# eragonruan/text-detection-ctpn

Hardware: NVIDIA H100
Metric: images/sec @600x900 (higher is better)
Workload: dtype fp32-faithful: fp16 operands + e4m3 cross terms (1 fp16 + 1 e4m3 wgmma per 16 MACs: 2 bf16-rate units per MAC), fp32 accumulate; matmuls around the BiLSTM on bf16x2

## Files before the change

text-detection-ctpn_b200/csrc/conv1_tc.cu:

```cuda
#include <mutex>

#include "common.cuh"
#include "tc_ptx.cuh"

namespace ctpn {

#ifdef CTPN_DEBUG
#define C1_DBG(p, bit) (((p).debug & (bit)) != 0)
#else
#define C1_DBG(p, bit) false
#endif


constexpr int kC1tThreads = 512;
constexpr int kC1tTileBytes = 128 * 128;
constexpr int kC1tPatch = 3 * 18 * 40;

struct Conv1TcParams {
  const void *src;
  const float *lut, *w, *bias;
  __nv_bfloat16 *out;
  int B, H, W, src_is_f32;
  int tiles_x, tiles_y, total_tiles;
  int debug;
  long long plane_stride;
  float out_s, out_t, out_rs;
  const int *sizes;
};

__device__ __forceinline__ void c1_extent(const Conv1TcParams &p, int b, int &eh, int &ew) {
  eh = p.H; ew = p.W;
  if (p.sizes) {
    eh = min(eh, __ldg(p.sizes + 2 * b));
    ew = min(ew, __ldg(p.sizes + 2 * b + 1));
  }
}

template <int P, int OUTQ>
__global__ void __launch_bounds__(kC1tThreads, 1)
conv1_tc_kernel(const Conv1TcParams p) {
  using namespace ptx;
  extern __shared__ uint8_t smem_raw[];
  const uint32_t raw = smem_u32(smem_raw);
  constexpr int kSPG = P <= 2 ? 2 : 1;
  constexpr int kStages = 2 * kSPG;
  const uint32_t a0 = (raw + 1023u) & ~1023u;
  const uint32_t b0 = a0 + (uint32_t)kStages * P * kC1tTileBytes;
  uint8_t *base = smem_raw + (a0 - raw);
  uint8_t *bsm = base + kStages * P * kC1tTileBytes;
  float *patch = reinterpret_cast<float *>(bsm + P * 64 * 128);
  float *lut_s = patch + 4 * kC1tPatch;
  float *epi = lut_s + 768;
  uint64_t *bars = reinterpret_cast<uint64_t *>(epi + 2 * 128 * 32);
  const uint32_t fullA = smem_u32(bars), emptyA = fullA + 32;

  const int warp = __shfl_sync(0xffffffffu, (int)(threadIdx.x >> 5), 0), lane = threadIdx.x & 31;
  if (threadIdx.x == 0) {
    for (int i = 0; i < 4; ++i) {
      mbar_init(fullA + 8 * i, 128);
      mbar_init(emptyA + 8 * i, 2);
    }
    fence_mbar_init();
  }
  if (!p.src_is_f32)
    for (int i = threadIdx.x; i < 768; i += kC1tThreads) lut_s[i] = p.lut[i];
  for (int i = threadIdx.x; i < 64 * 4; i += kC1tThreads) {
    const int co = i >> 2, chunk = i & 3;
    uint32_t pk[3][4];
#pragma unroll
    for (int j = 0; j < 4; ++j) {
      float v[2];
#pragma unroll
      for (int e = 0; e < 2; ++e) {
        const int k = chunk * 8 + j * 2 + e;
        v[e] = k < 27 ? p.w[k * 64 + co] : (k == 27 ? p.bias[co] : 0.f);
      }
      uint32_t t[P];
      split_planes2<P>(v[0], v[1], t);
#pragma unroll
      for (int pl = 0; pl < P; ++pl) pk[pl][j] = t[pl];
    }
#pragma unroll
    for (int pl = 0; pl < P; ++pl)
      *reinterpret_cast<uint4 *>(bsm + pl * 64 * 128 + co * 128 + ((chunk ^ (co & 7)) << 4)) = make_uint4(pk[pl][0], pk[pl][1], pk[pl][2], pk[pl][3]);
  }
  fence_proxy_async();
  __syncthreads();
  const int tiles_per_img = p.tiles_x * p.tiles_y;

  if (warp < 8) {
    const int grp = warp >> 2;
    const int m = (warp & 3) * 32 + lane, th = m >> 3, tw = m & 7;
    const unsigned tpi = (unsigned)tiles_per_img, tx = (unsigned)p.tiles_x;
    uint32_t raw[2][3];
    unsigned valid = 0;
    auto fetch = [&](int tile) {
      valid = 0;
      if (tile >= p.total_tiles) return;
      const unsigned b = (unsigned)tile / tpi, r = (unsigned)tile % tpi;
      const int y0 = (int)(r / tx) * 16, x0 = (int)(r % tx) * 8;
      int eh, ew;
      c1_extent(p, (int)b, eh, ew);
#pragma unroll
      for (int u = 0; u < 2; ++u) {
        const int i = m + u * 128;
        const int xx = i % 10, yy = i / 10;
        const int gx = x0 + xx - 1, gy = y0 + yy - 1;
        if (i < 180 && gx >= 0 && gx < ew && gy >= 0 && gy < eh && !C1_DBG(p, 1)) {
          const size_t off = (((size_t)b * p.H + gy) * p.W + gx) * 3;
          if (p.src_is_f32) {
            const float *q = reinterpret_cast<const float *>(p.src) + off;
            raw[u][0] = __float_as_uint(q[0]); raw[u][1] = __float_as_uint(q[1]); raw[u][2] = __float_as_uint(q[2]);
          } else {
            const uint8_t *q = reinterpret_cast<const uint8_t *>(p.src) + off;
            raw[u][0] = q[0]; raw[u][1] = q[1]; raw[u][2] = q[2];
          }
          valid |= 1u << u;
        }
      }
    };
    fetch(blockIdx.x + grp * gridDim.x);
    int n = 0;
    for (int tile = blockIdx.x + grp * gridDim.x; tile < p.total_tiles; tile += 2 * gridDim.x, ++n) {
      const int s = grp * kSPG + n % kSPG;
      const uint32_t ph = (uint32_t)(n / kSPG) & 1u;
      float *pt = patch + (grp * 2 + (n & 1)) * kC1tPatch;
#pragma unroll
      for (int u = 0; u < 2; ++u) {
        const int i = m + u * 128;
        if (i < 180) {
          const int xx = i % 10, yy = i / 10;
          float v0 = 0.f, v1 = 0.f, v2 = 0.f;
          if ((valid >> u) & 1u) {
            if (p.src_is_f32) {
              v0 = __uint_as_float(raw[u][0]); v1 = __uint_as_float(raw[u][1]); v2 = __uint_as_float(raw[u][2]);
            } else {
              v0 = lut_s[raw[u][0] * 3 + 0]; v1 = lut_s[raw[u][1] * 3 + 1]; v2 = lut_s[raw[u][2] * 3 + 2];
            }
          }
          pt[(0 * 18 + yy) * 40 + xx] = v0;
          pt[(1 * 18 + yy) * 40 + xx] = v1;
          pt[(2 * 18 + yy) * 40 + xx] = v2;
        }
      }
      fetch(tile + 2 * gridDim.x);
      mbar_wait(emptyA + 8 * s, ph ^ 1u);
      if (grp == 0) asm volatile("bar.sync 1, 128;" ::: "memory");
      else asm volatile("bar.sync 2, 128;" ::: "memory");
      uint8_t *arow = base + s * P * kC1tTileBytes + m * 128;
#pragma unroll
      for (int chunk = 0; chunk < (C1_DBG(p, 2) ? 0 : 4); ++chunk) {
        uint32_t pk[3][4];
#pragma unroll
        for (int j = 0; j < 4; ++j) {
          float v[2];
#pragma unroll
          for (int e = 0; e < 2; ++e) {
            const int k = chunk * 8 + j * 2 + e;
            v[e] = k < 27 ? pt[((k % 3) * 18 + th + k / 9) * 40 + tw + (k / 3) % 3] : (k == 27 ? 1.f : 0.f);
          }
          uint32_t t[P];
          split_planes2<P>(v[0], v[1], t);
#pragma unroll
          for (int pl = 0; pl < P; ++pl) pk[pl][j] = t[pl];
        }
#pragma unroll
        for (int pl = 0; pl < P; ++pl)
          *reinterpret_cast<uint4 *>(arow + pl * kC1tTileBytes + ((chunk ^ (m & 7)) << 4)) = make_uint4(pk[pl][0], pk[pl][1], pk[pl][2], pk[pl][3]);
      }
      fence_proxy_async();
      mbar_arrive(fullA + 8 * s);
    }
  } else {
    const int wg = (warp >> 2) - 2;
    const int cw = warp - 8, chunk = cw >> 2, quarter = cw & 3;
    const int m = quarter * 32 + lane, th = m >> 3, tw = m & 7;
    const int frow = wg * 64 + (warp & 3) * 16 + (lane >> 2);
    constexpr uint32_t kHi = gmma_desc_hi(1024);
    const uint32_t b_lo = gmma_desc_lo(b0);
    float accm[32], accc[32];
    uint4 *stage_w = reinterpret_cast<uint4 *>(epi + chunk * 4096 + quarter * 1024);
    int n = 0;
    for (int tile = blockIdx.x; tile < p.total_tiles; tile += gridDim.x, ++n) {
      const int s = (n & 1) * kSPG + (n >> 1) % kSPG;
      const uint32_t ph = (uint32_t)((n >> 1) / kSPG) & 1u;
      const unsigned b = (unsigned)tile / (unsigned)tiles_per_img, r = (unsigned)tile % (unsigned)tiles_per_img;
      const int y = (int)(r / (unsigned)p.tiles_x) * 16 + th, x = (int)(r % (unsigned)p.tiles_x) * 8 + tw;
      const bool ok = y < p.H && x < p.W;
      int eh, ew;
      c1_extent(p, (int)b, eh, ew);
      const bool live = y < eh && x < ew;
      const long long pix = ((long long)b * p.H + y) * p.W + x;
      const unsigned okmask = __ballot_sync(0xffffffffu, ok);
      long long spix[4];
#pragma unroll
      for (int it = 0; it < 4; ++it) {
        const long long hi = __shfl_sync(0xffffffffu, (int)(pix >> 32), it * 8 + (lane >> 2));
        const unsigned lo = __shfl_sync(0xffffffffu, (unsigned)(pix & 0xffffffffll), it * 8 + (lane >> 2));
        spix[it] = (hi << 32) | lo;
      }
      mbar_wait(fullA + 8 * s, ph);
      const uint32_t a_lo = gmma_desc_lo(a0 + s * P * kC1tTileBytes + wg * 64 * 128);
      wgmma_fence();
#pragma unroll
      for (int i = 0; i < P; ++i)
#pragma unroll
        for (int j = 0; j < P - i; ++j)
#pragma unroll
          for (int k = 0; k < 2; ++k) {
            const uint64_t da = ((uint64_t)kHi << 32) | (a_lo + i * (kC1tTileBytes >> 4) + 2u * k);
            const uint64_t db = ((uint64_t)kHi << 32) | (b_lo + j * ((64 * 128) >> 4) + 2u * k);
            if (i + j == 0) wgmma_bf16(accm, da, db, (uint32_t)k);
            else wgmma_bf16(accc, da, db, (k == 0 && i == 0 && j == 1) ? 0u : 1u);
          }
      wgmma_commit();
      wgmma_wait<0>();
      wgmma_fence_regs(accm);
      if (P > 1) wgmma_fence_regs(accc);
      if ((threadIdx.x & 127) == 0) mbar_arrive(emptyA + 8 * s);
      if (P > 1) {
#pragma unroll
        for (int i = 0; i < 32; ++i) accm[i] = accm[i] + accc[i];
      }
      named_sync(3, 256);
#pragma unroll
      for (int j = 0; j < 8; ++j) {
        const int q = 2 * (j & 3) + ((lane & 3) >> 1);
#pragma unroll
        for (int h = 0; h < 2; ++h) {
          const int row = frow + 8 * h;
          *reinterpret_cast<float2 *>(epi + (j >> 2) * 4096 + row * 32 + ((q ^ (row & 7)) << 2) + 2 * (lane & 1)) =
              make_float2(accm[4 * j + 2 * h], accm[4 * j + 2 * h + 1]);
        }
      }
      named_sync(3, 256);
      if (!C1_DBG(p, 8)) {
        float v[32];
#pragma unroll
        for (int q = 0; q < 8; ++q) {
          const float4 t = *reinterpret_cast<const float4 *>(epi + chunk * 4096 + m * 32 + ((q ^ (m & 7)) << 2));
          v[4 * q + 0] = t.x; v[4 * q + 1] = t.y; v[4 * q + 2] = t.z; v[4 * q + 3] = t.w;
        }
        if (!live) {
#pragma unroll
          for (int i = 0; i < 32; ++i) v[i] = 0.f;
        }
        if (OUTQ) {
          uint32_t wh[16], wq[16];
#pragma unroll
          for (int i = 0; i < 8; ++i) {
            const float v0 = fmaxf(v[4 * i], 0.f), v1 = fmaxf(v[4 * i + 1], 0.f), v2 = fmaxf(v[4 * i + 2], 0.f), v3 = fmaxf(v[4 * i + 3], 0.f);
            f16f8_quad(v0, v1, v2, v3, p.out_s, p.out_t, p.out_rs, wh[2 * i], wh[2 * i + 1], wq[i], wq[8 + i]);
          }
#pragma unroll
          for (int pl = 0; pl < 2; ++pl) {
            __syncwarp();
#pragma unroll
            for (int q = 0; q < 4; ++q) {
              const uint4 val = pl == 0 ? make_uint4(wh[4 * q], wh[4 * q + 1], wh[4 * q + 2], wh[4 * q + 3])
                                        : make_uint4(wq[4 * q], wq[4 * q + 1], wq[4 * q + 2], wq[4 * q + 3]);
              stage_w[lane * 4 + (q ^ ((lane >> 1) & 3))] = val;
            }
            __syncwarp();
            uint8_t *obase = reinterpret_cast<uint8_t *>(p.out) + (long long)pl * p.plane_stride * 2;
            const int j = lane & 3;
            const int off = pl == 0 ? chunk * 64 + j * 16 : chunk * 32 + (j >> 1) * 64 + (j & 1) * 16;
#pragma unroll
            for (int it = 0; it < 4; ++it) {
              const int pp = it * 8 + (lane >> 2);
              const uint4 val = stage_w[pp * 4 + (j ^ ((pp >> 1) & 3))];
              if (((okmask >> pp) & 1u) && !C1_DBG(p, 4)) *reinterpret_cast<uint4 *>(obase + spix[it] * 128 + off) = val;
            }
          }
        } else {
        uint32_t w[P][16];
#pragma unroll
        for (int i = 0; i < 16; ++i) {
          uint32_t t[P];
          split_planes2<P>(fmaxf(v[2 * i], 0.f), fmaxf(v[2 * i + 1], 0.f), t);
#pragma unroll
          for (int pl = 0; pl < P; ++pl) w[pl][i] = t[pl];
        }
#pragma unroll
        for (int pl = 0; pl < P; ++pl) {
          __syncwarp();
#pragma unroll
          for (int q = 0; q < 4; ++q) stage_w[lane * 4 + (q ^ ((lane >> 1) & 3))] = make_uint4(w[pl][4 * q], w[pl][4 * q + 1], w[pl][4 * q + 2], w[pl][4 * q + 3]);
          __syncwarp();
          __nv_bfloat16 *obase = p.out + (long long)pl * p.plane_stride + chunk * 32 + (lane & 3) * 8;
#pragma unroll
          for (int it = 0; it < 4; ++it) {
            const int pp = it * 8 + (lane >> 2);
            const uint4 val = stage_w[pp * 4 + ((lane & 3) ^ ((pp >> 1) & 3))];
            if (((okmask >> pp) & 1u) && !C1_DBG(p, 4)) *reinterpret_cast<uint4 *>(obase + spix[it] * 64) = val;
          }
        }
        }
      }
    }
  }
}

template <int P, int OUTQ = 0>
static int launch_conv1_tc(Conv1TcParams &p, cudaStream_t st) {
  const size_t smem = 1024 + (size_t)(P <= 2 ? 4 : 2) * P * kC1tTileBytes + (size_t)P * 64 * 128 +
                      (4 * kC1tPatch + 768 + 2 * 128 * 32) * sizeof(float) + 64;
  constexpr int kMaxDevices = 64;
  static std::mutex mu;
  static int sm_count[kMaxDevices];
  int dev = 0;
  CTPN_CUDA(cudaGetDevice(&dev));
  CTPN_REQUIRE(dev >= 0 && dev < kMaxDevices, "ctpn_conv1_1_tc: device index %d not supported", dev);
  int sms;
  {
    std::lock_guard<std::mutex> lock(mu);
    if (sm_count[dev] == 0) {
      CTPN_CUDA(cudaFuncSetAttribute(conv1_tc_kernel<P, OUTQ>, cudaFuncAttributeMaxDynamicSharedMemorySize, (int)smem));
      CTPN_CUDA(cudaDeviceGetAttribute(&sm_count[dev], cudaDevAttrMultiProcessorCount, dev));
    }
    sms = sm_count[dev];
  }
  const int grid = p.total_tiles < sms ? p.total_tiles : sms;
  ProfScope prof("conv1_1", 2.0 * p.B * p.H * p.W * 27.0 * 64.0, st);
  conv1_tc_kernel<P, OUTQ><<<grid, kC1tThreads, smem, st>>>(p);
  CTPN_LAUNCH_CHECK();
  return CTPN_OK;
}

}

int ctpn::conv1_1_tc_ragged(const void *src, int src_is_f32, const float *lut, const float *w_hwio, const float *bias,
                            void *out_planes, int B, int H, int W, int planes, bool outq, float out_s, float out_t,
                            const int *sizes, void *stream) {
  CTPN_REQUIRE(src && w_hwio && bias && out_planes, "ctpn_conv1_1_tc: null pointer");
  CTPN_REQUIRE(src_is_f32 || lut, "ctpn_conv1_1_tc: uint8 input needs the mean-subtraction LUT");
  CTPN_REQUIRE(B > 0 && H > 0 && W > 0, "ctpn_conv1_1_tc: bad shape");
  CTPN_REQUIRE(planes >= 1 && planes <= 3, "ctpn_conv1_1_tc: planes must be 1..3");
  Conv1TcParams p;
  p.src = src; p.lut = lut; p.w = w_hwio; p.bias = bias; p.out = (__nv_bfloat16 *)out_planes;
  p.B = B; p.H = H; p.W = W; p.src_is_f32 = src_is_f32;
  p.tiles_x = ceil_div(W, 8); p.tiles_y = ceil_div(H, 16);
  const long long total = (long long)B * p.tiles_x * p.tiles_y;
  CTPN_REQUIRE(total < (1ll << 31), "ctpn_conv1_1_tc: too many tiles");
  p.total_tiles = (int)total;
  p.plane_stride = (long long)B * H * W * 64;
  p.out_s = p.out_t = p.out_rs = 1.f;
  p.sizes = sizes;
  if (outq) {
    CTPN_REQUIRE(out_s > 0.f && out_t > 0.f, "ctpn_conv1_1_tc_f16f8: scales must be positive");
    p.out_s = out_s; p.out_t = out_t; p.out_rs = kResidualGain * out_t / out_s;
  }
#ifdef CTPN_DEBUG
  static const int dbg = [] { const char *e = getenv("CTPN_C1_DEBUG"); return e ? atoi(e) : 0; }();
  p.debug = dbg;
#else
  p.debug = 0;
#endif
  cudaStream_t st = (cudaStream_t)stream;
  if (outq) return launch_conv1_tc<2, 1>(p, st);
  if (planes == 1) return launch_conv1_tc<1>(p, st);
  if (planes == 2) return launch_conv1_tc<2>(p, st);
  return launch_conv1_tc<3>(p, st);
}

using namespace ctpn;

extern "C" int ctpn_conv1_1_tc(const void *src, int src_is_f32, const float *lut, const float *w_hwio, const float *bias,
                               void *out_planes, int B, int H, int W, int planes, void *stream) {
  return conv1_1_tc_ragged(src, src_is_f32, lut, w_hwio, bias, out_planes, B, H, W, planes, false, 1.f, 1.f, nullptr, stream);
}

extern "C" int ctpn_conv1_1_tc_f16f8(const void *src, int src_is_f32, const float *lut, const float *w_hwio, const float *bias,
                                     void *out_planes, int B, int H, int W, float out_s, float out_t, void *stream) {
  return conv1_1_tc_ragged(src, src_is_f32, lut, w_hwio, bias, out_planes, B, H, W, 2, true, out_s, out_t, nullptr, stream);
}
```

text-detection-ctpn_b200/csrc/conv_tc.cu:

```cuda
#include <cuda.h>

#include <algorithm>
#include <mutex>
#include <unordered_map>

#include "common.cuh"
#include "tc_ptx.cuh"
#include "tma_host.cuh"

namespace ctpn {

#ifdef CTPN_DEBUG
#define CTPN_DBG(p, bit) (((p).debug & (bit)) != 0)
#else
#define CTPN_DBG(p, bit) false
#endif

struct ConvTcParams {
  int B, H, W, Cin, Cout, taps, planes, flags;
  int tiles_x, tiles_y, tiles_n, total_tiles;
  int m_tiles, total_units;
  int TH, TW, tw_log2;
  int PW;
  int patch_bytes;
// ... 443 lines not shown
#pragma unroll
        for (int i = 0; i < R; ++i)
          accm[i] = F8 ? __fmaf_rn(accc[i], p.inv_cross, accm[i] * p.inv_main) : PR ? __fadd_rn(accs[i], accc[i]) : accm[i] + accc[i];
      }

      if (CTPN_DBG(p, 16)) continue;
      if (EW) {
        const float *bt = p.bias + (u % p.tiles_n) * BN + 2 * (lane & 3);
#pragma unroll
        for (int i8 = 0; i8 < BN / 8; ++i8) {
          const float2 bq = __ldg(reinterpret_cast<const float2 *>(bt + 8 * i8));
#pragma unroll
          for (int h = 0; h < 2; ++h) {
            accm[4 * i8 + 2 * h] += bq.x;
            accm[4 * i8 + 2 * h + 1] += bq.y;
          }
        }
        if (p.flags & CTPN_F_RELU) {
#pragma unroll
          for (int i = 0; i < R; ++i) accm[i] = fmaxf(accm[i], 0.f);
        }
#pragma unroll
        for (int c2 = 0; c2 < BN / 64; ++c2) {
          mbar_wait(epiE, eph ^ 1u);
          stage_half(c2);
          mbar_arrive(epiF);
          eph ^= 1u;
        }
      } else {
        const int cw = warp - 4, eset = cw >> 2, quarter = cw & 3;
        const int m = quarter * 32 + lane;
        int mt, nt;
        unit_tile(u, mt, nt);
        EpiPixel e;
        epi_pixel(p, mt, m, lane, e);
        uint4 *stage_w = reinterpret_cast<uint4 *>(epi + eset * 4096 + quarter * 1024);
#pragma unroll
        for (int c2 = 0; c2 < BN / 64; ++c2) {
          named_sync(1, 256);
          stage_half(c2);
          named_sync(1, 256);
          float v[32];
#pragma unroll
          for (int q = 0; q < 8; ++q) {
            const float4 t = *reinterpret_cast<const float4 *>(epi + eset * 4096 + m * 32 + ((q ^ (m & 7)) << 2));
            v[4 * q + 0] = t.x; v[4 * q + 1] = t.y; v[4 * q + 2] = t.z; v[4 * q + 3] = t.w;
          }
          epi_chunk<P, F8>(p, e, v, nt * BN + (2 * c2 + eset) * 32, stage_w, false, true, lane);
        }
      }
    }
  }
  __syncthreads();
  if (MC) cluster_sync_all();
}


constexpr int kMaxDevices = 64;
static std::mutex g_mu;
static int g_sms[kMaxDevices];

struct Tuning { int debug = 0, bn = 0, stages_a = 0, stages_b = 0, mcast = 1, promote = 1; };
static const Tuning &tuning() {
  static const Tuning t = [] {
    Tuning v;
#ifdef CTPN_DEBUG
    auto env_int = [](const char *name, int dflt) { const char *e = getenv(name); return e ? atoi(e) : dflt; };
    v.debug = env_int("CTPN_TC_DEBUG", 0);
    v.bn = env_int("CTPN_TC_BN", 0);
    v.stages_a = env_int("CTPN_TC_STAGES_A", 0);
    v.stages_b = env_int("CTPN_TC_STAGES_B", 0);
    v.mcast = env_int("CTPN_TC_MCAST", 1);
    v.promote = std::max(1, env_int("CTPN_TC_PROMOTE", 1));
#endif
    return v;
  }();
  return t;
}

struct TmapKey {
  const void *ptr;
  unsigned long long d0, d1, d2, d3;
  unsigned b0, b1, b2, b3;
  int dev;
  bool operator==(const TmapKey &o) const {
    return ptr == o.ptr && d0 == o.d0 && d1 == o.d1 && d2 == o.d2 && d3 == o.d3 && b0 == o.b0 && b1 == o.b1 && b2 == o.b2 &&
           b3 == o.b3 && dev == o.dev;
  }
};
struct TmapKeyHash {
  size_t operator()(const TmapKey &k) const {
    size_t h = std::hash<const void *>()(k.ptr);
    for (unsigned long long v : {k.d0, k.d1, k.d2, k.d3, (unsigned long long)k.b0, (unsigned long long)k.b1,
                                 (unsigned long long)k.b2, (unsigned long long)k.b3, (unsigned long long)k.dev})
      h = h * 1000003u ^ std::hash<unsigned long long>()(v);
    return h;
  }
};
static std::unordered_map<TmapKey, CUtensorMap, TmapKeyHash> g_tmaps;

static int cached_tmap(int dev, CUtensorMap *out, const void *ptr, int rank, const cuuint64_t *dims, const cuuint64_t *strides,
                       const cuuint32_t *box) {
  TmapKey k{ptr, dims[0], dims[1], rank > 2 ? dims[2] : 0, rank > 3 ? dims[3] : 0, box[0], box[1], rank > 2 ? box[2] : 0,
            rank > 3 ? box[3] : 0, dev};
  std::lock_guard<std::mutex> lock(g_mu);
  auto it = g_tmaps.find(k);
  if (it != g_tmaps.end()) { *out = it->second; return CTPN_OK; }
  EncodeTiledFn enc = nullptr;
  int rc = tma_get_encode(&enc);
  if (rc) return rc;
  if ((rc = tma_encode_bf16(enc, out, const_cast<void *>(ptr), rank, dims, strides, box))) return rc;
  if (g_tmaps.size() >= 1024) g_tmaps.clear();
  g_tmaps.emplace(k, *out);
  return CTPN_OK;
}

template <int BN, int P, int TAPS, int MC, int F8 = 0, int PR = 0>
static int launch_bn(int dev, const CUtensorMap &ta, const CUtensorMap &tb, ConvTcParams &p, cudaStream_t st) {
  const size_t a_stage = (size_t)p.planes * p.patch_bytes, b_stage = (size_t)p.planes * BN * 128;
  const size_t epi_bytes = kEpiBytes + (kEpiWarpgroup<BN, PR> ? kXposeBytes : 0);
  const size_t budget = 227 * 1024 - 1024 - kCtrlBytes - epi_bytes;
  int sa = (2 * a_stage + 2 * b_stage <= budget) ? 2 : 1;
  if (p.taps == 1) sa = (int)std::min<size_t>(4, std::max<size_t>(1, (budget / 2) / a_stage));
  CTPN_REQUIRE(sa * a_stage + 2 * b_stage <= budget, "conv_tc: pipeline stages (%zu + 2 x %zu B) do not fit in shared memory", a_stage, b_stage);
  int sb = (int)((budget - sa * a_stage) / b_stage);
  if (sb > kMaxStages) sb = kMaxStages;
  if (tuning().stages_a > 0) sa = std::max(1, std::min(sa, tuning().stages_a));
  if (tuning().stages_b > 0) sb = std::max(2, std::min(sb, tuning().stages_b));
  p.stages_a = sa;
  p.stages_b = sb;
  const size_t smem = 1024 + sa * a_stage + sb * b_stage + epi_bytes + kCtrlBytes;
  CTPN_REQUIRE(smem <= 227 * 1024, "conv_tc: %zu bytes of shared memory", smem);
  auto kernel = conv_tc_kernel<BN, P, TAPS, MC, F8, PR>;
  static bool attr_set[kMaxDevices];
  static int max_clusters[kMaxDevices];
  cudaLaunchConfig_t cfg = {};
  cudaLaunchAttribute attr;
  attr.id = cudaLaunchAttributeClusterDimension;
  attr.val.clusterDim.x = 2; attr.val.clusterDim.y = 1; attr.val.clusterDim.z = 1;
  cfg.blockDim = dim3(kTcThreads<BN, PR>);
  cfg.dynamicSmemBytes = smem;
  cfg.stream = st;
  cfg.attrs = &attr;
  cfg.numAttrs = MC ? 1 : 0;
  {
    std::lock_guard<std::mutex> lock(g_mu);
    if (!attr_set[dev]) {
      CTPN_CUDA(cudaFuncSetAttribute(kernel, cudaFuncAttributeMaxDynamicSharedMemorySize, 227 * 1024));
      if (MC) {
        cfg.gridDim = dim3(2 * (g_sms[dev] / 2));
        int n = 0;
        CTPN_CUDA(cudaOccupancyMaxActiveClusters(&n, kernel, &cfg));
        CTPN_REQUIRE(n > 0, "conv_tc: no 2-CTA cluster of this kernel fits on the device");
        max_clusters[dev] = n;
      }
      attr_set[dev] = true;
    }
  }
  char label[128];
  if (prof_enabled()) snprintf(label, sizeof(label), "conv_tc t%d %dx%dx%d c%d-%d %s%d bn%d%s%s", p.taps, p.B, p.H, p.W, p.Cin, p.Cout, F8 ? "f16f8 p" : "p", p.planes, BN, MC ? " mc" : "", PR ? " promote" : "");
  ProfScope prof(label, p.work, st);
  if (MC) cfg.gridDim = dim3(2 * std::min(max_clusters[dev], p.total_units));
  else cfg.gridDim = dim3(std::min(p.total_units, g_sms[dev]));
  CTPN_CUDA(cudaLaunchKernelEx(&cfg, kernel, ta, tb, p));
  CTPN_LAUNCH_CHECK();
  return CTPN_OK;
}

int conv_tc_run(const void *in_planes, const void *w_planes, const float *bias, void *out, int B, int H, int W, int cin,
                int cout, int taps, int planes, int flags, const QuantScales *q, const int *ext, int ext_shift, void *stream) {
  const bool f8 = q != nullptr, promote = (flags & CTPN_F_PROMOTE) != 0;
  CTPN_REQUIRE(f8 || !(flags & CTPN_F_OUT_BF16X2), "ctpn_conv3x3: CTPN_F_OUT_BF16X2 is a flag of ctpn_conv3x3_f16f8");
  CTPN_REQUIRE(!(promote && f8), "ctpn_conv3x3_f16f8: CTPN_F_PROMOTE is a flag of ctpn_conv3x3 with planes = 3");
  CTPN_REQUIRE(!promote || planes == 3, "ctpn_conv3x3: CTPN_F_PROMOTE needs planes = 3 (got %d)", planes);
  CTPN_REQUIRE(in_planes && w_planes && bias && out, "ctpn_conv3x3: null pointer");
  CTPN_REQUIRE(taps == 9 || taps == 1, "ctpn_conv3x3: taps must be 9 or 1 (got %d)", taps);
  CTPN_REQUIRE(planes >= 1 && planes <= 3, "ctpn_conv3x3: planes must be 1..3 (got %d)", planes);
  CTPN_REQUIRE(cin % 64 == 0 && cin >= 64, "ctpn_conv3x3: Cin must be a multiple of 64 (got %d)", cin);
  CTPN_REQUIRE(cout % 64 == 0 && cout >= 64, "ctpn_conv3x3: Cout must be a multiple of 64 (got %d)", cout);
  CTPN_REQUIRE(B > 0 && H > 0 && W > 0, "ctpn_conv3x3: bad shape");
  const bool pool = flags & CTPN_F_POOL;
  CTPN_REQUIRE(!pool || (taps == 9 && H >= 2 && W >= 2), "ctpn_conv3x3: pooling needs taps=9 and H,W >= 2");
  const bool stack_in = flags & CTPN_F_STACK_IN, stack_out = flags & CTPN_F_STACK_OUT;
  CTPN_REQUIRE(!stack_in || (taps == 9 && !pool), "ctpn_conv3x3: CTPN_F_STACK_IN needs taps=9 and no pooling");
  CTPN_REQUIRE(!stack_out || !(flags & CTPN_F_OUT_F32), "ctpn_conv3x3: stacked output is a plane format");
  const int img_B = B, img_H = H;
  if (stack_in) {
    CTPN_REQUIRE((long long)B * (H + 1) < (1ll << 30), "ctpn_conv3x3: stack too tall");
    H = B * (H + 1);
    B = 1;
  }
  int dev = 0, rc;
  CTPN_CUDA(cudaGetDevice(&dev));
  CTPN_REQUIRE(dev >= 0 && dev < kMaxDevices, "ctpn_conv3x3: device index %d not supported", dev);
// ... 130 lines not shown
```

text-detection-ctpn_b200/csrc/tc_ptx.cuh:

```cuda
#pragma once
#include <cuda.h>
#include <stdint.h>

namespace ctpn {
namespace ptx {

__device__ __forceinline__ uint32_t smem_u32(const void *p) {
  return static_cast<uint32_t>(__cvta_generic_to_shared(p));
}

__device__ __forceinline__ bool elect_one() {
  uint32_t pred = 0;
  asm volatile(
      "{\n\t.reg .pred p;\n\t"
      "elect.sync _|p, 0xffffffff;\n\t"
      "selp.u32 %0, 1, 0, p;\n\t}"
      : "=r"(pred));
  return pred != 0;
}

__device__ __forceinline__ void mbar_init(uint32_t bar, uint32_t count) {
  asm volatile("mbarrier.init.shared::cta.b64 [%0], %1;" ::"r"(bar), "r"(count) : "memory");
}
__device__ __forceinline__ void fence_mbar_init() {
  asm volatile("fence.mbarrier_init.release.cluster;" ::: "memory");
}
__device__ __forceinline__ void fence_proxy_async() {
  asm volatile("fence.proxy.async.shared::cta;" ::: "memory");
}
__device__ __forceinline__ void mbar_arrive_expect_tx(uint32_t bar, uint32_t bytes) {
  asm volatile("mbarrier.arrive.expect_tx.shared::cta.b64 _, [%0], %1;" ::"r"(bar), "r"(bytes) : "memory");
}
__device__ __forceinline__ void mbar_arrive(uint32_t bar) {
  asm volatile("mbarrier.arrive.shared::cta.b64 _, [%0];" ::"r"(bar) : "memory");
}
__device__ __forceinline__ bool mbar_try_wait(uint32_t bar, uint32_t parity) {
  uint32_t ok;
  asm volatile(
      "{\n\t.reg .pred p;\n\t"
      "mbarrier.try_wait.parity.shared::cta.b64 p, [%1], %2;\n\t"
      "selp.u32 %0, 1, 0, p;\n\t}"
      : "=r"(ok)
      : "r"(bar), "r"(parity)
      : "memory");
  return ok != 0;
}
__device__ __forceinline__ void mbar_wait(uint32_t bar, uint32_t parity) {
  if (mbar_try_wait(bar, parity)) return;
  const long long t0 = clock64();
  while (!mbar_try_wait(bar, parity)) {
    if (clock64() - t0 > 4000000000LL) __trap();
  }
}

__device__ __forceinline__ void prefetch_tmap(const CUtensorMap *m) {
  asm volatile("prefetch.tensormap [%0];" ::"l"(reinterpret_cast<uint64_t>(m)) : "memory");
}
__device__ __forceinline__ void tma_load_2d(const CUtensorMap *m, uint32_t bar, uint32_t dst, int c0, int c1) {
  asm volatile(
      "cp.async.bulk.tensor.2d.shared::cluster.global.mbarrier::complete_tx::bytes [%0], [%1, {%3, %4}], [%2];"
      ::"r"(dst), "l"(reinterpret_cast<uint64_t>(m)), "r"(bar), "r"(c0), "r"(c1)
      : "memory");
}
__device__ __forceinline__ void tma_load_4d(const CUtensorMap *m, uint32_t bar, uint32_t dst, int c0, int c1, int c2, int c3) {
  asm volatile(
      "cp.async.bulk.tensor.4d.shared::cluster.global.mbarrier::complete_tx::bytes [%0], [%1, {%3, %4, %5, %6}], [%2];"
      ::"r"(dst), "l"(reinterpret_cast<uint64_t>(m)), "r"(bar), "r"(c0), "r"(c1), "r"(c2), "r"(c3)
      : "memory");
}

__device__ __forceinline__ void tma_load_2d_mc(const CUtensorMap *m, uint32_t bar, uint32_t dst, int c0, int c1, uint16_t cta_mask) {
  asm volatile(
      "cp.async.bulk.tensor.2d.shared::cluster.global.mbarrier::complete_tx::bytes.multicast::cluster [%0], [%1, {%4, %5}], [%2], %3;"
      ::"r"(dst), "l"(reinterpret_cast<uint64_t>(m)), "r"(bar), "h"(cta_mask), "r"(c0), "r"(c1)
      : "memory");
}

__device__ __forceinline__ void cluster_sync_all() {
  asm volatile("barrier.cluster.arrive.release.aligned;\n\tbarrier.cluster.wait.acquire.aligned;" ::: "memory");
}
__device__ __forceinline__ uint32_t cluster_ctarank() {
  uint32_t r;
  asm volatile("mov.u32 %0, %%cluster_ctarank;" : "=r"(r));
  return r;
}

__device__ __forceinline__ void mbar_arrive_cluster(uint32_t bar, uint32_t cta) {
  asm volatile(
      "{\n\t.reg .b32 ra;\n\t"
      "mapa.shared::cluster.u32 ra, %0, %1;\n\t"
      "mbarrier.arrive.release.cluster.shared::cluster.b64 _, [ra];\n\t}"
      ::"r"(bar), "r"(cta) : "memory");
}

__device__ __forceinline__ void named_sync(uint32_t id, uint32_t count) {
  asm volatile("bar.sync %0, %1;" ::"r"(id), "r"(count) : "memory");
}

template <uint32_t R> __device__ __forceinline__ void regs_dealloc() { asm volatile("setmaxnreg.dec.sync.aligned.u32 %0;" ::"n"(R)); }
template <uint32_t R> __device__ __forceinline__ void regs_alloc() { asm volatile("setmaxnreg.inc.sync.aligned.u32 %0;" ::"n"(R)); }

__device__ __forceinline__ void wgmma_fence() { asm volatile("wgmma.fence.sync.aligned;" ::: "memory"); }
__device__ __forceinline__ void wgmma_commit() { asm volatile("wgmma.commit_group.sync.aligned;" ::: "memory"); }
template <int N> __device__ __forceinline__ void wgmma_wait() { asm volatile("wgmma.wait_group.sync.aligned %0;" ::"n"(N) : "memory"); }
template <int R> __device__ __forceinline__ void wgmma_fence_regs(float (&d)[R]) {
#pragma unroll
  for (int i = 0; i < R; ++i) asm volatile("" : "+f"(d[i])::"memory");
}

__host__ __device__ constexpr uint32_t gmma_desc_hi(uint32_t stride_bytes) { return (stride_bytes >> 4) | (1u << 30); }
__device__ __forceinline__ uint32_t gmma_desc_lo(uint32_t smem_addr) { return ((smem_addr >> 4) & 0x3FFFu) | (1u << 16); }

#define CTPN_WGMMA_N64(NAME, KTYPE, TRANS)                                                                   \
  __device__ __forceinline__ void NAME(float (&d)[32], uint64_t da, uint64_t db, uint32_t acc) {              \
    asm volatile("{\n\t.reg .pred p;\n\tsetp.ne.b32 p, %34, 0;\n\t"                                          \
                 "wgmma.mma_async.sync.aligned.m64n64" KTYPE " {%0, %1, %2, %3, %4, %5, %6, %7, %8, %9, %10, %11, %12, %13, %14, %15, %16, %17, %18, %19, %20, %21, %22, %23, %24, %25, %26, %27, %28, %29, %30, %31}, %32, %33, p, 1, 1" TRANS ";\n\t}" \
                 : "+f"(d[0]), "+f"(d[1]), "+f"(d[2]), "+f"(d[3]), "+f"(d[4]), "+f"(d[5]), "+f"(d[6]), "+f"(d[7]), "+f"(d[8]), "+f"(d[9]), "+f"(d[10]), "+f"(d[11]), "+f"(d[12]), "+f"(d[13]), "+f"(d[14]), "+f"(d[15]), "+f"(d[16]), "+f"(d[17]), "+f"(d[18]), "+f"(d[19]), "+f"(d[20]), "+f"(d[21]), "+f"(d[22]), "+f"(d[23]), "+f"(d[24]), "+f"(d[25]), "+f"(d[26]), "+f"(d[27]), "+f"(d[28]), "+f"(d[29]), "+f"(d[30]), "+f"(d[31]) \
                 : "l"(da), "l"(db), "r"(acc));                                                      \
  }
#define CTPN_WGMMA_N128(NAME, KTYPE, TRANS)                                                                   \
  __device__ __forceinline__ void NAME(float (&d)[64], uint64_t da, uint64_t db, uint32_t acc) {              \
    asm volatile("{\n\t.reg .pred p;\n\tsetp.ne.b32 p, %66, 0;\n\t"                                          \
                 "wgmma.mma_async.sync.aligned.m64n128" KTYPE " {%0, %1, %2, %3, %4, %5, %6, %7, %8, %9, %10, %11, %12, %13, %14, %15, %16, %17, %18, %19, %20, %21, %22, %23, %24, %25, %26, %27, %28, %29, %30, %31, %32, %33, %34, %35, %36, %37, %38, %39, %40, %41, %42, %43, %44, %45, %46, %47, %48, %49, %50, %51, %52, %53, %54, %55, %56, %57, %58, %59, %60, %61, %62, %63}, %64, %65, p, 1, 1" TRANS ";\n\t}" \
                 : "+f"(d[0]), "+f"(d[1]), "+f"(d[2]), "+f"(d[3]), "+f"(d[4]), "+f"(d[5]), "+f"(d[6]), "+f"(d[7]), "+f"(d[8]), "+f"(d[9]), "+f"(d[10]), "+f"(d[11]), "+f"(d[12]), "+f"(d[13]), "+f"(d[14]), "+f"(d[15]), "+f"(d[16]), "+f"(d[17]), "+f"(d[18]), "+f"(d[19]), "+f"(d[20]), "+f"(d[21]), "+f"(d[22]), "+f"(d[23]), "+f"(d[24]), "+f"(d[25]), "+f"(d[26]), "+f"(d[27]), "+f"(d[28]), "+f"(d[29]), "+f"(d[30]), "+f"(d[31]), "+f"(d[32]), "+f"(d[33]), "+f"(d[34]), "+f"(d[35]), "+f"(d[36]), "+f"(d[37]), "+f"(d[38]), "+f"(d[39]), "+f"(d[40]), "+f"(d[41]), "+f"(d[42]), "+f"(d[43]), "+f"(d[44]), "+f"(d[45]), "+f"(d[46]), "+f"(d[47]), "+f"(d[48]), "+f"(d[49]), "+f"(d[50]), "+f"(d[51]), "+f"(d[52]), "+f"(d[53]), "+f"(d[54]), "+f"(d[55]), "+f"(d[56]), "+f"(d[57]), "+f"(d[58]), "+f"(d[59]), "+f"(d[60]), "+f"(d[61]), "+f"(d[62]), "+f"(d[63]) \
                 : "l"(da), "l"(db), "r"(acc));                                                      \
  }
#define CTPN_WGMMA_N256(NAME, KTYPE, TRANS)                                                                   \
  __device__ __forceinline__ void NAME(float (&d)[128], uint64_t da, uint64_t db, uint32_t acc) {              \
    asm volatile("{\n\t.reg .pred p;\n\tsetp.ne.b32 p, %130, 0;\n\t"                                          \
                 "wgmma.mma_async.sync.aligned.m64n256" KTYPE " {%0, %1, %2, %3, %4, %5, %6, %7, %8, %9, %10, %11, %12, %13, %14, %15, %16, %17, %18, %19, %20, %21, %22, %23, %24, %25, %26, %27, %28, %29, %30, %31, %32, %33, %34, %35, %36, %37, %38, %39, %40, %41, %42, %43, %44, %45, %46, %47, %48, %49, %50, %51, %52, %53, %54, %55, %56, %57, %58, %59, %60, %61, %62, %63, %64, %65, %66, %67, %68, %69, %70, %71, %72, %73, %74, %75, %76, %77, %78, %79, %80, %81, %82, %83, %84, %85, %86, %87, %88, %89, %90, %91, %92, %93, %94, %95, %96, %97, %98, %99, %100, %101, %102, %103, %104, %105, %106, %107, %108, %109, %110, %111, %112, %113, %114, %115, %116, %117, %118, %119, %120, %121, %122, %123, %124, %125, %126, %127}, %128, %129, p, 1, 1" TRANS ";\n\t}" \
                 : "+f"(d[0]), "+f"(d[1]), "+f"(d[2]), "+f"(d[3]), "+f"(d[4]), "+f"(d[5]), "+f"(d[6]), "+f"(d[7]), "+f"(d[8]), "+f"(d[9]), "+f"(d[10]), "+f"(d[11]), "+f"(d[12]), "+f"(d[13]), "+f"(d[14]), "+f"(d[15]), "+f"(d[16]), "+f"(d[17]), "+f"(d[18]), "+f"(d[19]), "+f"(d[20]), "+f"(d[21]), "+f"(d[22]), "+f"(d[23]), "+f"(d[24]), "+f"(d[25]), "+f"(d[26]), "+f"(d[27]), "+f"(d[28]), "+f"(d[29]), "+f"(d[30]), "+f"(d[31]), "+f"(d[32]), "+f"(d[33]), "+f"(d[34]), "+f"(d[35]), "+f"(d[36]), "+f"(d[37]), "+f"(d[38]), "+f"(d[39]), "+f"(d[40]), "+f"(d[41]), "+f"(d[42]), "+f"(d[43]), "+f"(d[44]), "+f"(d[45]), "+f"(d[46]), "+f"(d[47]), "+f"(d[48]), "+f"(d[49]), "+f"(d[50]), "+f"(d[51]), "+f"(d[52]), "+f"(d[53]), "+f"(d[54]), "+f"(d[55]), "+f"(d[56]), "+f"(d[57]), "+f"(d[58]), "+f"(d[59]), "+f"(d[60]), "+f"(d[61]), "+f"(d[62]), "+f"(d[63]), "+f"(d[64]), "+f"(d[65]), "+f"(d[66]), "+f"(d[67]), "+f"(d[68]), "+f"(d[69]), "+f"(d[70]), "+f"(d[71]), "+f"(d[72]), "+f"(d[73]), "+f"(d[74]), "+f"(d[75]), "+f"(d[76]), "+f"(d[77]), "+f"(d[78]), "+f"(d[79]), "+f"(d[80]), "+f"(d[81]), "+f"(d[82]), "+f"(d[83]), "+f"(d[84]), "+f"(d[85]), "+f"(d[86]), "+f"(d[87]), "+f"(d[88]), "+f"(d[89]), "+f"(d[90]), "+f"(d[91]), "+f"(d[92]), "+f"(d[93]), "+f"(d[94]), "+f"(d[95]), "+f"(d[96]), "+f"(d[97]), "+f"(d[98]), "+f"(d[99]), "+f"(d[100]), "+f"(d[101]), "+f"(d[102]), "+f"(d[103]), "+f"(d[104]), "+f"(d[105]), "+f"(d[106]), "+f"(d[107]), "+f"(d[108]), "+f"(d[109]), "+f"(d[110]), "+f"(d[111]), "+f"(d[112]), "+f"(d[113]), "+f"(d[114]), "+f"(d[115]), "+f"(d[116]), "+f"(d[117]), "+f"(d[118]), "+f"(d[119]), "+f"(d[120]), "+f"(d[121]), "+f"(d[122]), "+f"(d[123]), "+f"(d[124]), "+f"(d[125]), "+f"(d[126]), "+f"(d[127]) \
                 : "l"(da), "l"(db), "r"(acc));                                                      \
  }

CTPN_WGMMA_N64(wgmma_bf16, "k16.f32.bf16.bf16", ", 0, 0")
CTPN_WGMMA_N128(wgmma_bf16, "k16.f32.bf16.bf16", ", 0, 0")
CTPN_WGMMA_N256(wgmma_bf16, "k16.f32.bf16.bf16", ", 0, 0")
CTPN_WGMMA_N64(wgmma_f16, "k16.f32.f16.f16", ", 0, 0")
CTPN_WGMMA_N128(wgmma_f16, "k16.f32.f16.f16", ", 0, 0")
CTPN_WGMMA_N256(wgmma_f16, "k16.f32.f16.f16", ", 0, 0")
CTPN_WGMMA_N64(wgmma_e4m3, "k32.f32.e4m3.e4m3", "")
CTPN_WGMMA_N128(wgmma_e4m3, "k32.f32.e4m3.e4m3", "")
CTPN_WGMMA_N256(wgmma_e4m3, "k32.f32.e4m3.e4m3", "")
#undef CTPN_WGMMA_N64
#undef CTPN_WGMMA_N128
#undef CTPN_WGMMA_N256

}
}
```

text-detection-ctpn_b200/csrc/tma_host.cuh:

```cuda
#pragma once
#include <cuda.h>

#include <mutex>

#include "common.cuh"

namespace ctpn {

typedef CUresult (*EncodeTiledFn)(CUtensorMap *, CUtensorMapDataType, cuuint32_t, void *, const cuuint64_t *,
                                  const cuuint64_t *, const cuuint32_t *, const cuuint32_t *, CUtensorMapInterleave,
                                  CUtensorMapSwizzle, CUtensorMapL2promotion, CUtensorMapFloatOOBfill);

inline int tma_get_encode(EncodeTiledFn *out) {
  static EncodeTiledFn fn = nullptr;
  static std::mutex mu;
  std::lock_guard<std::mutex> lock(mu);
  if (!fn) {
    void *sym = nullptr;
    cudaDriverEntryPointQueryResult qres;
    CTPN_CUDA(cudaGetDriverEntryPoint("cuTensorMapEncodeTiled", &sym, cudaEnableDefault, &qres));
    if (!sym || qres != cudaDriverEntryPointSuccess) {
      set_error("cuTensorMapEncodeTiled is not available from this driver");
      return CTPN_ERR_CUDA;
    }
    fn = reinterpret_cast<EncodeTiledFn>(sym);
  }
  *out = fn;
  return CTPN_OK;
}

inline int tma_encode_bf16(EncodeTiledFn fn, CUtensorMap *m, void *addr, int rank, const cuuint64_t *dims,
                           const cuuint64_t *strides, const cuuint32_t *box) {
  cuuint32_t ones[5] = {1, 1, 1, 1, 1};
  CUresult r = fn(m, CU_TENSOR_MAP_DATA_TYPE_BFLOAT16, rank, addr, dims, strides, box, ones, CU_TENSOR_MAP_INTERLEAVE_NONE,
                  CU_TENSOR_MAP_SWIZZLE_128B, CU_TENSOR_MAP_L2_PROMOTION_L2_256B, CU_TENSOR_MAP_FLOAT_OOB_FILL_NONE);
  if (r != CUDA_SUCCESS) {
    set_error("cuTensorMapEncodeTiled failed with CUresult %d (rank %d)", (int)r, rank);
    return CTPN_ERR_CUDA;
  }
  return CTPN_OK;
}

}
```

Before: 813.1.

## Write conv1_1 epilogue output via TMA bulk tensor stores

Replaces the per-lane 16-byte global stores in the conv1_1 tensor-core epilogue with 4D TMA tensor stores from swizzled shared-memory boxes, one per plane per warp. A bulk-group wait before each reuse of the staging buffer lets the stores overlap the next tile's MMA. The tensor-map cache now takes the data type and swizzle mode as part of its key. Bounds masking moves to TMA's out-of-range clipping, and the smem layout is reordered so the epilogue buffer stays aligned for swizzled boxes.

Measured after the change: 815.9 (median of 6 runs). No clear change (+0.3%).

```diff
diff --git a/text-detection-ctpn_b200/csrc/conv1_tc.cu b/text-detection-ctpn_b200/csrc/conv1_tc.cu
--- a/text-detection-ctpn_b200/csrc/conv1_tc.cu
+++ b/text-detection-ctpn_b200/csrc/conv1_tc.cu
@@ -2,6 +2,7 @@
 
 #include "common.cuh"
 #include "tc_ptx.cuh"
+#include "tma_host.cuh"
 
 namespace ctpn {
 
@@ -38,7 +39,8 @@
 
 template <int P, int OUTQ>
 __global__ void __launch_bounds__(kC1tThreads, 1)
-conv1_tc_kernel(const Conv1TcParams p) {
+conv1_tc_kernel(const __grid_constant__ CUtensorMap tmap_o0, const __grid_constant__ CUtensorMap tmap_o1,
+                const Conv1TcParams p) {
   using namespace ptx;
   extern __shared__ uint8_t smem_raw[];
   const uint32_t raw = smem_u32(smem_raw);
@@ -48,14 +50,16 @@
   const uint32_t b0 = a0 + (uint32_t)kStages * P * kC1tTileBytes;
   uint8_t *base = smem_raw + (a0 - raw);
   uint8_t *bsm = base + kStages * P * kC1tTileBytes;
-  float *patch = reinterpret_cast<float *>(bsm + P * 64 * 128);
+  float *epi = reinterpret_cast<float *>(bsm + P * 64 * 128);
+  float *patch = epi + 2 * 128 * 32;
   float *lut_s = patch + 4 * kC1tPatch;
-  float *epi = lut_s + 768;
-  uint64_t *bars = reinterpret_cast<uint64_t *>(epi + 2 * 128 * 32);
+  uint64_t *bars = reinterpret_cast<uint64_t *>(lut_s + 768);
   const uint32_t fullA = smem_u32(bars), emptyA = fullA + 32;
 
   const int warp = __shfl_sync(0xffffffffu, (int)(threadIdx.x >> 5), 0), lane = threadIdx.x & 31;
   if (threadIdx.x == 0) {
+    prefetch_tmap(&tmap_o0);
+    if (OUTQ) prefetch_tmap(&tmap_o1);
     for (int i = 0; i < 4; ++i) {
       mbar_init(fullA + 8 * i, 128);
       mbar_init(emptyA + 8 * i, 2);
@@ -179,26 +183,18 @@
     constexpr uint32_t kHi = gmma_desc_hi(1024);
     const uint32_t b_lo = gmma_desc_lo(b0);
     float accm[32], accc[32];
-    uint4 *stage_w = reinterpret_cast<uint4 *>(epi + chunk * 4096 + quarter * 1024);
+    uint8_t *box = reinterpret_cast<uint8_t *>(epi + chunk * 4096 + quarter * 1024);
+    const uint32_t box_s = smem_u32(box);
     int n = 0;
     for (int tile = blockIdx.x; tile < p.total_tiles; tile += gridDim.x, ++n) {
       const int s = (n & 1) * kSPG + (n >> 1) % kSPG;
       const uint32_t ph = (uint32_t)((n >> 1) / kSPG) & 1u;
       const unsigned b = (unsigned)tile / (unsigned)tiles_per_img, r = (unsigned)tile % (unsigned)tiles_per_img;
-      const int y = (int)(r / (unsigned)p.tiles_x) * 16 + th, x = (int)(r % (unsigned)p.tiles_x) * 8 + tw;
-      const bool ok = y < p.H && x < p.W;
+      const int y0 = (int)(r / (unsigned)p.tiles_x) * 16, x0 = (int)(r % (unsigned)p.tiles_x) * 8;
+      const int y = y0 + th, x = x0 + tw;
       int eh, ew;
       c1_extent(p, (int)b, eh, ew);
       const bool live = y < eh && x < ew;
-      const long long pix = ((long long)b * p.H + y) * p.W + x;
-      const unsigned okmask = __ballot_sync(0xffffffffu, ok);
-      long long spix[4];
-#pragma unroll
-      for (int it = 0; it < 4; ++it) {
-        const long long hi = __shfl_sync(0xffffffffu, (int)(pix >> 32), it * 8 + (lane >> 2));
-        const unsigned lo = __shfl_sync(0xffffffffu, (unsigned)(pix & 0xffffffffll), it * 8 + (lane >> 2));
-        spix[it] = (hi << 32) | lo;
-      }
       mbar_wait(fullA + 8 * s, ph);
       const uint32_t a_lo = gmma_desc_lo(a0 + s * P * kC1tTileBytes + wg * 64 * 128);
       wgmma_fence();
@@ -222,6 +218,7 @@
 #pragma unroll
         for (int i = 0; i < 32; ++i) accm[i] = accm[i] + accc[i];
       }
+      if (lane == 0) bulk_wait_read<0>();
       named_sync(3, 256);
 #pragma unroll
       for (int j = 0; j < 8; ++j) {
@@ -245,6 +242,13 @@
 #pragma unroll
           for (int i = 0; i < 32; ++i) v[i] = 0.f;
         }
+        __syncwarp();
+        auto put16 = [&](int slot, const uint32_t *w) {
+#pragma unroll
+          for (int q = 0; q < 4; ++q)
+            *reinterpret_cast<uint4 *>(box + slot * 2048 + lane * 64 + ((q ^ ((lane >> 1) & 3)) << 4)) = make_uint4(w[4 * q], w[4 * q + 1], w[4 * q + 2], w[4 * q + 3]);
+        };
+        const int ys = y0 + quarter * 4;
         if (OUTQ) {
           uint32_t wh[16], wq[16];
 #pragma unroll
@@ -252,52 +256,48 @@
             const float v0 = fmaxf(v[4 * i], 0.f), v1 = fmaxf(v[4 * i + 1], 0.f), v2 = fmaxf(v[4 * i + 2], 0.f), v3 = fmaxf(v[4 * i + 3], 0.f);
             f16f8_quad(v0, v1, v2, v3, p.out_s, p.out_t, p.out_rs, wh[2 * i], wh[2 * i + 1], wq[i], wq[8 + i]);
           }
-#pragma unroll
-          for (int pl = 0; pl < 2; ++pl) {
+          put16(0, wh);
+#pragma unroll
+          for (int h = 0; h < 2; ++h)
+#pragma unroll
+            for (int q = 0; q < 2; ++q)
+              *reinterpret_cast<uint4 *>(box + 2048 + h * 1024 + lane * 32 + ((q ^ ((lane >> 2) & 1)) << 4)) =
+                  make_uint4(wq[8 * h + 4 * q], wq[8 * h + 4 * q + 1], wq[8 * h + 4 * q + 2], wq[8 * h + 4 * q + 3]);
+          fence_proxy_async();
+          __syncwarp();
+          if (lane == 0 && !C1_DBG(p, 4)) {
+            tma_store_4d(&tmap_o0, box_s, chunk * 32, x0, ys, (int)b);
+            tma_store_4d(&tmap_o1, box_s + 2048, chunk * 32, x0, ys, (int)b);
+            tma_store_4d(&tmap_o1, box_s + 3072, 64 + chunk * 32, x0, ys, (int)b);
+            bulk_commit();
+          }
+        } else {
+          uint32_t w[P][16];
+#pragma unroll
+          for (int i = 0; i < 16; ++i) {
+            uint32_t t[P];
+            split_planes2<P>(fmaxf(v[2 * i], 0.f), fmaxf(v[2 * i + 1], 0.f), t);
+#pragma unroll
+            for (int pl = 0; pl < P; ++pl) w[pl][i] = t[pl];
+          }
+#pragma unroll
+          for (int pl = 0; pl < P; ++pl) {
+            if (pl >= 2) {
+              if (lane == 0) bulk_wait_read<1>();
+              __syncwarp();
+            }
+            put16(pl & 1, w[pl]);
+            fence_proxy_async();
             __syncwarp();
-#pragma unroll
-            for (int q = 0; q < 4; ++q) {
-              const uint4 val = pl == 0 ? make_uint4(wh[4 * q], wh[4 * q + 1], wh[4 * q + 2], wh[4 * q + 3])
-                                        : make_uint4(wq[4 * q], wq[4 * q + 1], wq[4 * q + 2], wq[4 * q + 3]);
-              stage_w[lane * 4 + (q ^ ((lane >> 1) & 3))] = val;
+            if (lane == 0 && !C1_DBG(p, 4)) {
+              tma_store_4d(&tmap_o0, box_s + (pl & 1) * 2048, chunk * 32, x0, ys, pl * p.B + (int)b);
+              bulk_commit();
             }
-            __syncwarp();
-            uint8_t *obase = reinterpret_cast<uint8_t *>(p.out) + (long long)pl * p.plane_stride * 2;
-            const int j = lane & 3;
-            const int off = pl == 0 ? chunk * 64 + j * 16 : chunk * 32 + (j >> 1) * 64 + (j & 1) * 16;
-#pragma unroll
-            for (int it = 0; it < 4; ++it) {
-              const int pp = it * 8 + (lane >> 2);
-              const uint4 val = stage_w[pp * 4 + (j ^ ((pp >> 1) & 3))];
-              if (((okmask >> pp) & 1u) && !C1_DBG(p, 4)) *reinterpret_cast<uint4 *>(obase + spix[it] * 128 + off) = val;
-            }
-          }
-        } else {
-        uint32_t w[P][16];
-#pragma unroll
-        for (int i = 0; i < 16; ++i) {
-          uint32_t t[P];
-          split_planes2<P>(fmaxf(v[2 * i], 0.f), fmaxf(v[2 * i + 1], 0.f), t);
-#pragma unroll
-          for (int pl = 0; pl < P; ++pl) w[pl][i] = t[pl];
-        }
-#pragma unroll
-        for (int pl = 0; pl < P; ++pl) {
-          __syncwarp();
-#pragma unroll
-          for (int q = 0; q < 4; ++q) stage_w[lane * 4 + (q ^ ((lane >> 1) & 3))] = make_uint4(w[pl][4 * q], w[pl][4 * q + 1], w[pl][4 * q + 2], w[pl][4 * q + 3]);
-          __syncwarp();
-          __nv_bfloat16 *obase = p.out + (long long)pl * p.plane_stride + chunk * 32 + (lane & 3) * 8;
-#pragma unroll
-          for (int it = 0; it < 4; ++it) {
-            const int pp = it * 8 + (lane >> 2);
-            const uint4 val = stage_w[pp * 4 + ((lane & 3) ^ ((pp >> 1) & 3))];
-            if (((okmask >> pp) & 1u) && !C1_DBG(p, 4)) *reinterpret_cast<uint4 *>(obase + spix[it] * 64) = val;
-          }
-        }
-        }
-      }
-    }
+          }
+        }
+      }
+    }
+    if (lane == 0) bulk_wait<0>();
   }
 }
 
@@ -320,9 +320,25 @@
     }
     sms = sm_count[dev];
   }
+  CUtensorMap t0, t1;
+  const cuuint64_t pix = (cuuint64_t)p.W * p.H;
+  const cuuint64_t dims[4] = {64, (cuuint64_t)p.W, (cuuint64_t)p.H, (cuuint64_t)(OUTQ ? 1 : P) * p.B};
+  const cuuint64_t strides[3] = {128, (cuuint64_t)p.W * 128, pix * 128};
+  const cuuint32_t box[4] = {32, 8, 4, 1};
+  int rc;
+  if ((rc = cached_tmap(dev, &t0, p.out, 4, dims, strides, box,
+                        OUTQ ? CU_TENSOR_MAP_DATA_TYPE_FLOAT16 : CU_TENSOR_MAP_DATA_TYPE_BFLOAT16, CU_TENSOR_MAP_SWIZZLE_64B)))
+    return rc;
+  t1 = t0;
+  if (OUTQ) {
+    const cuuint64_t dq[4] = {128, (cuuint64_t)p.W, (cuuint64_t)p.H, (cuuint64_t)p.B};
+    if ((rc = cached_tmap(dev, &t1, p.out + p.plane_stride, 4, dq, strides, box, CU_TENSOR_MAP_DATA_TYPE_UINT8,
+                          CU_TENSOR_MAP_SWIZZLE_32B)))
+      return rc;
+  }
   const int grid = p.total_tiles < sms ? p.total_tiles : sms;
   ProfScope prof("conv1_1", 2.0 * p.B * p.H * p.W * 27.0 * 64.0, st);
-  conv1_tc_kernel<P, OUTQ><<<grid, kC1tThreads, smem, st>>>(p);
+  conv1_tc_kernel<P, OUTQ><<<grid, kC1tThreads, smem, st>>>(t0, t1, p);
   CTPN_LAUNCH_CHECK();
   return CTPN_OK;
 }
@@ -336,6 +352,7 @@
   CTPN_REQUIRE(src_is_f32 || lut, "ctpn_conv1_1_tc: uint8 input needs the mean-subtraction LUT");
   CTPN_REQUIRE(B > 0 && H > 0 && W > 0, "ctpn_conv1_1_tc: bad shape");
   CTPN_REQUIRE(planes >= 1 && planes <= 3, "ctpn_conv1_1_tc: planes must be 1..3");
+  CTPN_REQUIRE(((uintptr_t)out_planes & 15) == 0, "ctpn_conv1_1_tc: the output must be 16-byte aligned");
   Conv1TcParams p;
   p.src = src; p.lut = lut; p.w = w_hwio; p.bias = bias; p.out = (__nv_bfloat16 *)out_planes;
   p.B = B; p.H = H; p.W = W; p.src_is_f32 = src_is_f32;
diff --git a/text-detection-ctpn_b200/csrc/conv_tc.cu b/text-detection-ctpn_b200/csrc/conv_tc.cu
--- a/text-detection-ctpn_b200/csrc/conv_tc.cu
+++ b/text-detection-ctpn_b200/csrc/conv_tc.cu
@@ -549,34 +549,35 @@
   const void *ptr;
   unsigned long long d0, d1, d2, d3;
   unsigned b0, b1, b2, b3;
-  int dev;
+  int dev, dt, sw;
   bool operator==(const TmapKey &o) const {
     return ptr == o.ptr && d0 == o.d0 && d1 == o.d1 && d2 == o.d2 && d3 == o.d3 && b0 == o.b0 && b1 == o.b1 && b2 == o.b2 &&
-           b3 == o.b3 && dev == o.dev;
+           b3 == o.b3 && dev == o.dev && dt == o.dt && sw == o.sw;
   }
 };
 struct TmapKeyHash {
   size_t operator()(const TmapKey &k) const {
     size_t h = std::hash<const void *>()(k.ptr);
     for (unsigned long long v : {k.d0, k.d1, k.d2, k.d3, (unsigned long long)k.b0, (unsigned long long)k.b1,
-                                 (unsigned long long)k.b2, (unsigned long long)k.b3, (unsigned long long)k.dev})
+                                 (unsigned long long)k.b2, (unsigned long long)k.b3, (unsigned long long)k.dev,
+                                 (unsigned long long)k.dt, (unsigned long long)k.sw})
       h = h * 1000003u ^ std::hash<unsigned long long>()(v);
     return h;
   }
 };
 static std::unordered_map<TmapKey, CUtensorMap, TmapKeyHash> g_tmaps;
 
-static int cached_tmap(int dev, CUtensorMap *out, const void *ptr, int rank, const cuuint64_t *dims, const cuuint64_t *strides,
-                       const cuuint32_t *box) {
+int cached_tmap(int dev, CUtensorMap *out, const void *ptr, int rank, const cuuint64_t *dims, const cuuint64_t *strides,
+                const cuuint32_t *box, CUtensorMapDataType dt, CUtensorMapSwizzle sw) {
   TmapKey k{ptr, dims[0], dims[1], rank > 2 ? dims[2] : 0, rank > 3 ? dims[3] : 0, box[0], box[1], rank > 2 ? box[2] : 0,
-            rank > 3 ? box[3] : 0, dev};
+            rank > 3 ? box[3] : 0, dev, (int)dt, (int)sw};
   std::lock_guard<std::mutex> lock(g_mu);
   auto it = g_tmaps.find(k);
   if (it != g_tmaps.end()) { *out = it->second; return CTPN_OK; }
   EncodeTiledFn enc = nullptr;
   int rc = tma_get_encode(&enc);
   if (rc) return rc;
-  if ((rc = tma_encode_bf16(enc, out, const_cast<void *>(ptr), rank, dims, strides, box))) return rc;
+  if ((rc = tma_encode(enc, out, const_cast<void *>(ptr), rank, dims, strides, box, dt, sw))) return rc;
   if (g_tmaps.size() >= 1024) g_tmaps.clear();
   g_tmaps.emplace(k, *out);
   return CTPN_OK;
diff --git a/text-detection-ctpn_b200/csrc/tc_ptx.cuh b/text-detection-ctpn_b200/csrc/tc_ptx.cuh
--- a/text-detection-ctpn_b200/csrc/tc_ptx.cuh
+++ b/text-detection-ctpn_b200/csrc/tc_ptx.cuh
@@ -68,6 +68,15 @@
       ::"r"(dst), "l"(reinterpret_cast<uint64_t>(m)), "r"(bar), "r"(c0), "r"(c1), "r"(c2), "r"(c3)
       : "memory");
 }
+
+__device__ __forceinline__ void tma_store_4d(const CUtensorMap *m, uint32_t src, int c0, int c1, int c2, int c3) {
+  asm volatile("cp.async.bulk.tensor.4d.global.shared::cta.bulk_group [%0, {%2, %3, %4, %5}], [%1];"
+               ::"l"(reinterpret_cast<uint64_t>(m)), "r"(src), "r"(c0), "r"(c1), "r"(c2), "r"(c3)
+               : "memory");
+}
+__device__ __forceinline__ void bulk_commit() { asm volatile("cp.async.bulk.commit_group;" ::: "memory"); }
+template <int N> __device__ __forceinline__ void bulk_wait_read() { asm volatile("cp.async.bulk.wait_group.read %0;" ::"n"(N) : "memory"); }
+template <int N> __device__ __forceinline__ void bulk_wait() { asm volatile("cp.async.bulk.wait_group %0;" ::"n"(N) : "memory"); }
 
 __device__ __forceinline__ void tma_load_2d_mc(const CUtensorMap *m, uint32_t bar, uint32_t dst, int c0, int c1, uint16_t cta_mask) {
   asm volatile(
diff --git a/text-detection-ctpn_b200/csrc/tma_host.cuh b/text-detection-ctpn_b200/csrc/tma_host.cuh
--- a/text-detection-ctpn_b200/csrc/tma_host.cuh
+++ b/text-detection-ctpn_b200/csrc/tma_host.cuh
@@ -29,11 +29,13 @@
   return CTPN_OK;
 }
 
-inline int tma_encode_bf16(EncodeTiledFn fn, CUtensorMap *m, void *addr, int rank, const cuuint64_t *dims,
-                           const cuuint64_t *strides, const cuuint32_t *box) {
+inline int tma_encode(EncodeTiledFn fn, CUtensorMap *m, void *addr, int rank, const cuuint64_t *dims,
+                      const cuuint64_t *strides, const cuuint32_t *box,
+                      CUtensorMapDataType dt = CU_TENSOR_MAP_DATA_TYPE_BFLOAT16,
+                      CUtensorMapSwizzle sw = CU_TENSOR_MAP_SWIZZLE_128B) {
   cuuint32_t ones[5] = {1, 1, 1, 1, 1};
-  CUresult r = fn(m, CU_TENSOR_MAP_DATA_TYPE_BFLOAT16, rank, addr, dims, strides, box, ones, CU_TENSOR_MAP_INTERLEAVE_NONE,
-                  CU_TENSOR_MAP_SWIZZLE_128B, CU_TENSOR_MAP_L2_PROMOTION_L2_256B, CU_TENSOR_MAP_FLOAT_OOB_FILL_NONE);
+  CUresult r = fn(m, dt, rank, addr, dims, strides, box, ones, CU_TENSOR_MAP_INTERLEAVE_NONE, sw,
+                  CU_TENSOR_MAP_L2_PROMOTION_L2_256B, CU_TENSOR_MAP_FLOAT_OOB_FILL_NONE);
   if (r != CUDA_SUCCESS) {
     set_error("cuTensorMapEncodeTiled failed with CUresult %d (rank %d)", (int)r, rank);
     return CTPN_ERR_CUDA;
@@ -41,4 +43,8 @@
   return CTPN_OK;
 }
 
+int cached_tmap(int dev, CUtensorMap *out, const void *ptr, int rank, const cuuint64_t *dims, const cuuint64_t *strides,
+                const cuuint32_t *box, CUtensorMapDataType dt = CU_TENSOR_MAP_DATA_TYPE_BFLOAT16,
+                CUtensorMapSwizzle sw = CU_TENSOR_MAP_SWIZZLE_128B);
+
 }
```
